# Parskatt/RoMa

Measured on AMD Instinct MI355X. Metric: image-pairs/sec, roma_outdoor 560->864, batch=8 per GPU, higher is better.
Workload: dtype bf16; 1 GPU; roma_outdoor match() 560->864, symmetric, upsample_preds, 8 pairs/GPU/step, seeded synthetic weights + N(0,1) images; precision policy of the reference's bf16 timing script: bfloat16 DINOv2 + float16 autocast for VGG / decoder / refiners (ROMA_MIXED), f32 accumulate; precision_policy=mixed, global_batch=8, streams_per_gpu=2, parallelism=single GPU, outputs_finite=True

## Files before the change

roma_amd/csrc/dwconv_ring.hip:

```cpp
#include <stdlib.h>

#include <algorithm>

#include "elementwise.h"
#include "tuning.h"
#include "gemm.h"

namespace roma {

typedef __attribute__((ext_vector_type(2))) float f32x2;
#define ROMA_LDS __attribute__((address_space(3)))
typedef ROMA_LDS unsigned char lds_u8;

__device__ __attribute__((aligned(256))) unsigned int g_dwr_zero_page[64];

constexpr int DWR_ROWB = 3072;
constexpr int DWR_PXW = 16;
constexpr int DWR_NR = 6;
constexpr int DWR_RING = 4 * DWR_NR * DWR_ROWB;
static_assert(3 * (DWR_NR - 1) + 4 * (DWR_NR - 1) <= 63, "vmcnt is a 6-bit counter");
static_assert(2 * DWR_RING <= 160 * 1024, "two workgroups per CU");

#define ROMA_DWR_WAIT_VM(N) asm volatile("s_waitcnt vmcnt(%0)" ::"n"(N) : "memory")

__device__ __forceinline__ void dwr_glds16(const char* src, lds_u8* lds_wave_base) {
  __builtin_amdgcn_global_load_lds((const __attribute__((address_space(1))) void*)src, (ROMA_LDS void*)lds_wave_base, 16, 0, 0);
}

__device__ __forceinline__ void dwr_read(unsigned long long (&cr)[8], unsigned rd) {
  asm volatile(
      "ds_read_b64 %0, %8\n\tds_read_b64 %1, %8 offset:128\n\tds_read_b64 %2, %8 offset:256\n\t"
      "ds_read_b64 %3, %8 offset:384\n\tds_read_b64 %4, %8 offset:640\n\tds_read_b64 %5, %8 offset:768\n\t"
      "ds_read_b64 %6, %8 offset:896\n\tds_read_b64 %7, %8 offset:1024"
      : "=&v"(cr[0]), "=&v"(cr[1]), "=&v"(cr[2]), "=&v"(cr[3]), "=&v"(cr[4]), "=&v"(cr[5]), "=&v"(cr[6]), "=&v"(cr[7])
      : "v"(rd)
      : "memory");
}
__device__ __forceinline__ void dwr_wait(unsigned long long (&cr)[8]) {
  asm volatile("s_waitcnt lgkmcnt(0)"
               : "+v"(cr[0]), "+v"(cr[1]), "+v"(cr[2]), "+v"(cr[3]), "+v"(cr[4]), "+v"(cr[5]), "+v"(cr[6]), "+v"(cr[7])::"memory");
}

__device__ __forceinline__ void dwr_row(f32x2 (&acc)[5][4][2], const f32x4 (&wreg)[25], f32x2 bias0, f32x2 bias1,
                                        unsigned long long (&cr)[8], unsigned rd_next, bool store, bf16_t* orow, long Cp, int npx) {
  f32x2 v[8][2];
#define ROMA_DWR_CVT(J)                                                  \
  {                                                                      \
    const uint32_t lo_ = (uint32_t)cr[J], hi_ = (uint32_t)(cr[J] >> 32); \
    v[J][0] = f32x2{h16_lo(lo_), h16_hi(lo_)};                           \
    v[J][1] = f32x2{h16_lo(hi_), h16_hi(hi_)};                           \
  }
  ROMA_DWR_CVT(0) ROMA_DWR_CVT(1) ROMA_DWR_CVT(2) ROMA_DWR_CVT(3) ROMA_DWR_CVT(4) ROMA_DWR_CVT(5) ROMA_DWR_CVT(6) ROMA_DWR_CVT(7)
#undef ROMA_DWR_CVT
#pragma unroll
  for (int j = 0; j < 8; ++j) asm volatile("" : "+v"(v[j][0]), "+v"(v[j][1]));
  dwr_read(cr, rd_next);
#pragma unroll
  for (int kx = 0; kx < 5; ++kx) {
    __builtin_amdgcn_sched_barrier(0);
#pragma unroll
    for (int k = 0; k < 5; ++k) {
      const f32x4 wx = wreg[(4 - k) * 5 + kx];
      const f32x2 w0 = f32x2{wx[0], wx[1]}, w1 = f32x2{wx[2], wx[3]};
#pragma unroll
      for (int px = 0; px < 4; ++px) {
        acc[k][px][0] = v[px + kx][0] * w0 + (k == 4 && kx == 0 ? bias0 : acc[k][px][0]);
        acc[k][px][1] = v[px + kx][1] * w1 + (k == 4 && kx == 0 ? bias1 : acc[k][px][1]);
      }
    }
    __builtin_amdgcn_sched_barrier(0);
  }
  if (store) {
#pragma unroll
    for (int px = 0; px < 4; ++px) {
      if (px < npx) {
        uint2 u;
        u.x = pack_relu_h16x2(acc[0][px][0][0], acc[0][px][0][1]);
        u.y = pack_relu_h16x2(acc[0][px][1][0], acc[0][px][1][1]);
        *reinterpret_cast<uint2*>(orow + (long)px * Cp) = u;
      }
    }
  }
#pragma unroll
  for (int k = 0; k < 4; ++k)
#pragma unroll
    for (int px = 0; px < 4; ++px) {
      acc[k][px][0] = acc[k + 1][px][0];
      acc[k][px][1] = acc[k + 1][px][1];
    }
  dwr_wait(cr);
}

__global__ __launch_bounds__(256, 2) void dwconv5x5_ring_kernel(const bf16_t* __restrict__ in, bf16_t* __restrict__ out,
                                                                const float* __restrict__ w, const float* __restrict__ bias,
                                                                int B, int H, int W, int Cp, int SY, int nchunk, int nxg,
                                                                long ntasks) {
  constexpr int NR = DWR_NR;
  __shared__ __attribute__((aligned(1024))) unsigned char ring[DWR_RING];
  const long nwg = (ntasks + 3) / 4, wg_per_xcd = (nwg + 7) / 8;
  const long lw = (long)(blockIdx.x % 8) * wg_per_xcd + blockIdx.x / 8;
  const int lane = threadIdx.x & 63;
  const int wv = __builtin_amdgcn_readfirstlane((int)(threadIdx.x >> 6));
  const long task = lw * 4 + wv;
  if (lw >= nwg || task >= ntasks) return;
  const int xg = (int)(task % nxg);
  long r = task / nxg;
  const int chunk = (int)(r % nchunk);
  r /= nchunk;
  const int yt = (H + SY - 1) / SY;
  const int ys = (int)(r % yt) * SY;
  const int b = (int)(r / yt);
  const int sy = min(SY, H - ys);
  const int T = sy + 4;

  const int cg = lane & 15, xq = lane >> 4;
  const int c = chunk * 64 + cg * 4;

  f32x4 wreg[25];
#pragma unroll
  for (int t = 0; t < 25; ++t) wreg[t] = *reinterpret_cast<const f32x4*>(w + (long)t * Cp + c);
  const f32x4 bx = *reinterpret_cast<const f32x4*>(bias + c);
#pragma unroll
  for (int t = 0; t < 25; ++t) asm volatile("" : "+v"(wreg[t]));
  const f32x2 bias0 = f32x2{bx[0], bx[1]}, bias1 = f32x2{bx[2], bx[3]};
  asm volatile("s_waitcnt vmcnt(0)" ::: "memory");

  const int xb = xg * DWR_PXW + xq * 4;
  const int x0 = xg * DWR_PXW - 2;
  const int npx = min(4, W - xb);

  const char* zsrc = reinterpret_cast<const char*>(g_dwr_zero_page);
  const char* inb = reinterpret_cast<const char*>(in + ((long)b * H * W) * Cp) + (long)chunk * 128;
  const long pitch = (long)W * Cp * 2;
  const __amdgpu_buffer_rsrc_t rs_in = __builtin_amdgcn_make_buffer_rsrc(const_cast<char*>(inb), 0, (int)((long)H * pitch - (long)chunk * 128), 0x00020000);
  unsigned voff[3];
#pragma unroll
  for (int i = 0; i < 3; ++i) {
    const int p = 64 * i + lane, s = p >> 3, part = p & 7;
    const int x = x0 + s - s / 5;
    const bool ok = (s % 5 != 4) && x >= 0 && x < W;
    voff[i] = ok ? (unsigned)(x * Cp * 2 + part * 16) : 0x80000000u;
  }
  unsigned vout = 0x80000000u;
  asm volatile("" : "+v"(vout));
  lds_u8* const myring = (lds_u8*)ring + wv * (NR * DWR_ROWB);
#define ROMA_DWR_BL16(VOFF, SOFF, DST) \
  __builtin_amdgcn_raw_ptr_buffer_load_lds(rs_in, (ROMA_LDS void*)(DST), 16, (int)(VOFF), (int)(SOFF), 0, 0)
#define ROMA_DWR_ISSUE(RROW, SLOT)                                                         \
  {                                                                                        \
    const int yy_ = ys - 2 + (RROW);                                                       \
    if ((RROW) < T && yy_ >= 0 && yy_ < H) {                             \
      const int so_ = yy_ * (int)pitch;                                                    \
      _Pragma("unroll") for (int i = 0; i < 3; ++i) ROMA_DWR_BL16(voff[i], so_, myring + (SLOT) * DWR_ROWB + i * 1024); \
    } else {                                                                               \
      _Pragma("unroll") for (int i = 0; i < 3; ++i) ROMA_DWR_BL16(vout, 0, myring + (SLOT) * DWR_ROWB + i * 1024); \
    }                                                                                      \
  }

  f32x2 acc[5][4][2];
#pragma unroll
  for (int s5 = 0; s5 < 5; ++s5)
#pragma unroll
    for (int px = 0; px < 4; ++px) {
      acc[s5][px][0] = bias0;
      acc[s5][px][1] = bias1;
    }
  const unsigned ring_lds = (unsigned)(size_t)myring;
  const unsigned rd0 = ring_lds + (unsigned)(xq * 5 * 128 + cg * 8);
  bf16_t* const obase = out + ((long)b * H * W) * Cp + c;

#pragma unroll
  for (int rr = 0; rr < NR - 1; ++rr) ROMA_DWR_ISSUE(rr, rr);
  unsigned long long cr[8];
  ROMA_DWR_WAIT_VM(3 * (NR - 2));
  dwr_read(cr, rd0);
  dwr_wait(cr);

  int slot1 = 1;
  int fill = NR - 1;
  bf16_t* orow = obase + ((long)ys * W + xb) * Cp;
  const long orow_step = (long)W * Cp;
#pragma nounroll
  for (int t = 0; t < T; ++t) {
    ROMA_DWR_ISSUE(t + NR - 1, fill);
    ROMA_DWR_WAIT_VM(3 * (NR - 2));
    const bool st = t >= 4;
    dwr_row(acc, wreg, bias0, bias1, cr, rd0 + (unsigned)slot1 * DWR_ROWB, st && npx > 0, orow, (long)Cp, npx);
    if (st) orow += orow_step;
    fill = fill + 1 == NR ? 0 : fill + 1;
    slot1 = slot1 + 1 == NR ? 0 : slot1 + 1;
  }
#undef ROMA_DWR_ISSUE
  ROMA_DWR_WAIT_VM(0);
}

int dwconv5x5_ring_try_launch(const void* in, void* out, const float* w, const float* bias, int B, int H, int W, int Cp, int dt,
                              hipStream_t s) {
  const int dw_ring = tuning(SW_DW_RING);
  if (!dw_ring) return 1;
  if (dt != DT_BF16 || Cp % 64 != 0 || Cp < 256 || H < 1 || W < 1) return 1;
  if ((long)H * W * Cp * 2 >= (1l << 31)) return 1;
  if ((reinterpret_cast<uintptr_t>(in) & 15) != 0 || (reinterpret_cast<uintptr_t>(out) & 7) != 0) return 1;
  if ((reinterpret_cast<uintptr_t>(w) & 15) != 0 || (reinterpret_cast<uintptr_t>(bias) & 15) != 0) return 1;
  const int nchunk = Cp / 64;
  const int nxg = (W + DWR_PXW - 1) / DWR_PXW;
  int SY = H;
  {
    long best = -1;
    const long per_strip = (long)B * nxg * nchunk;
    const int max_sy = std::max(6, (int)tuning(SW_DWR_MAXSY));
    for (int ns = (H + max_sy - 1) / max_sy; ns <= std::max(1, H / 6); ++ns) {
      const int sy = (H + ns - 1) / ns;
      const long nt = per_strip * ((H + sy - 1) / sy);
      const long cost = ((nt + 2047) / 2048) * (sy + 7);
      if (best < 0 || cost < best) {
        best = cost;
        SY = sy;
      }
    }
  }
  const long ntasks = (long)B * ((H + SY - 1) / SY) * nxg * nchunk;
  ROMA_REQUIRE(ntasks < (1l << 31), "dwconv5x5: grid too large");
  const long min_elems = tuning(SW_DW_RING_MINELEMS);
  if (dw_ring != 2 && (long)B * H * W * Cp < min_elems) return 1;
  ProfScope ps("dwconv5x5_kernel<" ROMA_H16_NAME ">", 2.0 * (double)B * H * W * Cp * 2.0, "byte", s);
  const long nwg = (ntasks + 3) / 4;
  hipLaunchKernelGGL(dwconv5x5_ring_kernel, dim3((unsigned)(((nwg + 7) / 8) * 8)), dim3(256), 0, s, (const bf16_t*)in,
                     (bf16_t*)out, w, bias, B, H, W, Cp, SY, nchunk, nxg, ntasks);
  ROMA_LAUNCH_CHECK();
  return 0;
}

}
```

roma_amd/csrc/elementwise.h:

```cpp
#pragma once
#include "common.h"

namespace roma {

int layernorm_launch(const float* x, const float* w, const float* b, void* out, long M, int D, float eps,
                     int dt_out, hipStream_t s);
int layernorm_launch_dt(const void* x, int dt_in, const float* w, const float* b, void* out, long M, int D, float eps,
                        int dt_out, hipStream_t s);

int conv3x3_c3_launch(const float* img, const float* w, const float* bias, void* out, int B, int H, int W,
                      int dt_out, hipStream_t s);

int im2col3x3_c3_launch(const float* img, void* out, int B, int H, int W, int dt_out, hipStream_t s);

int maxpool2x2_launch(const void* in, void* out, int B, int H, int W, int C, int dt, hipStream_t s);

int im2col_patch14_launch(const float* img, void* out, int B, int H, int W, int Kpad, int dt_out, hipStream_t s);

int assemble_tokens_launch(const float* patch, const float* cls, const float* pos, float* tokens, int B, int T,
                           int D, hipStream_t s);

int copy2d_launch(const void* in, long ldi, int dt_in, void* out, long ldo, int dt_out, long rows, int cols,
                  hipStream_t s);

int convert_from_bf16_launch(const void* in, void* out, long n, hipStream_t s);

int rownorm_launch(const void* in, long ld, int dt, float* norms, long M, int C, hipStream_t s);

int gp_basis_launch(const float* w, const float* b, float* Ft, int Dg, int h, int wdt, int npad, hipStream_t s, int copies = 1,
                    long stride = 0);

int transpose_launch(const float* in, float* out, int n, long ld, int batch, hipStream_t s, long stride_in = 0, long stride_out = 0);

int chol_diag_launch(float* A, long ld, long strideA, float* Linv, float* LinvT, int k, int nblk, int batch,
                     hipStream_t s);

int chol_col_launch(float* A, long ld, long strideA, float* LT, long strideLT, int n, int d, float* Linv, float* LinvT, int k,
                    int nblk, int batch, unsigned epoch, int use_leader, hipStream_t s);
int chol_col_restore_launch(float* A, long ld, long strideA, const float* LT, long strideLT, int n, int batch, hipStream_t s);

int pad_identity_launch(float* A, long ld, long strideA, int n, int npad, int batch, hipStream_t s);

int cls_to_flow_launch(const float* logits, long ld, float* flow, float* cert, long M, hipStream_t s);

struct RefinerInputArgs {
  const void* feat = nullptr;
  long ldf = 0;
  const float* flow = nullptr;
  void* d = nullptr;
  long ldd = 0;
  const float* emb_w = nullptr;
  const float* emb_b = nullptr;
  int B = 0, H = 0, W = 0, C = 0, E = 0, Kcorr = 0, nimg = 0, shift = 0;
  float disp_scale = 1.f;
  int dt = 0;
};
int refiner_input_launch(const RefinerInputArgs& a, hipStream_t s);

int dwconv5x5_launch(const void* in, void* out, const float* w, const float* bias, int B, int H, int W, int Cp,
                     int dt, hipStream_t s);
int dwconv5x5_ring_try_launch(const void* in, void* out, const float* w, const float* bias, int B, int H, int W, int Cp, int dt,
                              hipStream_t s);

int refiner_out_launch(const void* d, long ldd, int dt, const float* w , const float* b ,
                       float* flow, float* cert, long M, int Cp, float sx, float sy, hipStream_t s);
int refiner_apply_delta_launch(const float* delta, float* flow, float* cert, long M, float sx, float sy, hipStream_t s);

int resize_bilinear_launch(const float* in, float* out, int B, int Hin, int Win, int Hout, int Wout, int nc,
                           hipStream_t s);

struct FinalArgs {
  const float* flow = nullptr;
  const float* cert = nullptr;
  const float* cert16 = nullptr;
  float* warp = nullptr;
  float* certainty = nullptr;
  int B = 0, H = 0, W = 0, h16 = 0, w16 = 0, symmetric = 1;
};
int final_epilogue_launch(const FinalArgs& a, hipStream_t s);

int checksum_cols_launch(const void* p, long rows, int ld, int c0, int c1, unsigned long long* out, hipStream_t s);
int checksum_launch(const void* p, size_t bytes, unsigned long long* out, hipStream_t s);

}
```

roma_amd/csrc/tuning.hip:

```cpp
#include "tuning.h"

#include <stdlib.h>
#include <string.h>

#include "../../include/roma_hip.h"

namespace roma {
void set_error(const std::string& msg);
namespace {

struct Row {
  Switch id;
  const char* key;
  const char* env;
  long def;
  int floor;
  const char* doc;
};

constexpr Row ROWS[] = {
    {SW_GEMM8P, "gemm8p", "ROMA_GEMM8P", 1, 0, "large bf16 GEMMs on the 8-phase 256 x 256 kernel (1) or on the one-barrier-per-slab kernel (0)"},
    {SW_GEMM_DBG, "gemm_dbg", "ROMA_GEMM_DBG", 0, 0, "experiment bits of the GEMM kernels (1 skip output stores, 2 skip the K loop, 2048 no streaming stores, ...)"},
    {SW_GEMM8P_WALK, "gemm8p_walk", nullptr, -1, 1, "gemm8p: tile rows per group of the persistent walk (1 = row major); unset = 8 from 24 tile columns on, else 1"},
    {SW_GEMM8P_SCHED, "gemm8p_sched", "ROMA_GEMM8P_SCHED", 1, 0, "gemm8p K-loop schedule: 1 k-half phases, 0 quadrant phases (tools builds only)"},
    {SW_GEMM8P_MAXWG, "gemm8p_maxwg", nullptr, -1, 8, "gemm8p, measurement only: cap the persistent grid at n workgroups (a multiple of 8); unset = one per CU"},
    {SW_WS1X1, "ws1x1", "ROMA_WS1X1", 1, 0, "N = K = 576 refiner 1x1 on the weight-stationary kernel (1) or on the 256 x 192 tile kernel (0)"},
    {SW_LC_MODE, "lc_mode", "ROMA_LC_MODE", 0, 0, "local correlation: 0 tiled form + gather work list, 1 every tile on the gather list (key only), 2 per-pixel kernel"},
    {SW_LC_BIN, "lc_bin", "ROMA_LC_BIN", 1, 0, "local correlation: queries of incoherent tiles sorted by target bin, counters in LDS (1) or device atomics (2), or gathered per query (0)"},
    {SW_CONV64, "conv64", "ROMA_CONV64", 7, 0, "weight-stationary VGG front end, bit mask: 1 the Cin = 64 kernels, 2 the Cin = 128 kernel, 4 the fused first layer"},
    {SW_CONV_PATCH, "conv_patch", "ROMA_CONV_PATCH", 1, 0, "patch-resident 3x3 kernel for slab-major VGG layers (1) or gemm8p (0); environment 0 also packs tap-major weights"},
    {SW_ATTN_XCD, "attn_xcd", "ROMA_ATTN_XCD", 1, 0, "attention work items in per-XCD bands of (batch, head) (1) or in plain order (0)"},
    {SW_ATTN_EXP2, "attn_exp2", nullptr, -1, 0, "tools only: force the 2^x softmax of the 16-bit attention kernel on / off; unset = as the caller says"},
    {SW_DW_RING, "dw_ring", "ROMA_DW_RING", 1, 0, "depthwise 5x5: 0 register-prefetch kernel, 1 ring kernel for the large launches, 2 ring kernel for every shape it takes"},
    {SW_GP_COL, "gp_col", "ROMA_GP_COL", 1, 0, "GP Cholesky left-looking, one launch per block column (1) or the right-looking launch chain (0)"},
    {SW_POOL_PROJ, "pool_proj", "ROMA_POOL_PROJ", 1, 0, "max-pool + proj head of strides 1 / 2 in one pass (1) or as separate kernels (0)"},
    {SW_GP_COL_LEADER, "gp_col_leader", "ROMA_GP_COL_LEADER", 1, 0, "block-column Cholesky: a leader workgroup factorises the diagonal block, its product formed one launch ahead (1) or in its own launch (2), or every workgroup its own copy (0)"},
    {SW_GEMM8P_MINM, nullptr, "ROMA_GEMM8P_MINM", 2048, 0, "gemm8p: smallest M it takes for the wide (N >= 2048) dense launches"},
    {SW_GEMM_NT, nullptr, "ROMA_GEMM_NT", 1, 0, "non-temporal output stores in the 16-bit GEMM row writer"},
    {SW_GEMM_F32_FILL, nullptr, "ROMA_GEMM_F32_FILL", 1, 0, "exact-f32 GEMMs below 192 tiles of 256 x 256 run on 128 x 128 tiles"},
    {SW_GEMM_SMALLM, nullptr, "ROMA_GEMM_SMALLM", 1, 0, "GEMMs below 320 tiles of 128 x 128 run on 128 x 64 tiles"},
    {SW_CONV64_SY, nullptr, "ROMA_CONV64_SY", 0, 0, "conv64 strip height in rows; 0 = the split of H with the fewest rounds"},
    {SW_CONV_KORDER, nullptr, "ROMA_CONV_KORDER", 1, 0, "VGG layers with Cout >= 256 pack slab-major weight rows (read when a handle is created)"},
    {SW_RB_SY, nullptr, "ROMA_RB_SY", 0, 0, "fused refiner block strip height in rows; 0 = the split of H with the fewest rounds"},
    {SW_DWR_MAXSY, nullptr, "ROMA_DWR_MAXSY", 1 << 20, 0, "depthwise ring kernel: cap of the strip height in rows (at least 6)"},
    {SW_DW_RING_MINELEMS, nullptr, "ROMA_DW_RING_MINELEMS", 64l << 20, 0, "dw_ring = 1: smallest launch, in elements, that goes to the ring kernel"},
    {SW_RI_VEC, nullptr, "ROMA_RI_VEC", 1, 0, "refiner_input on the 16-byte vector kernel where alignment allows"},
    {SW_OUT_ROW, nullptr, "ROMA_OUT_ROW", 1, 0, "refiner_out: row kernel for C = 24 in 16-bit storage"},
    {SW_OUT_LPR, nullptr, "ROMA_OUT_LPR", 1, 0, "refiner_out, 16-bit: lanes per row chosen to fill the 16-byte pieces best"},
    {SW_OUT_ROWS_IT, nullptr, "ROMA_OUT_ROWS_IT", 0, 0, "refiner_out: row groups per wave (even, >= 2); otherwise 8"},
    {SW_GP_AUG, nullptr, "ROMA_GP_AUG", 1, 0, "GP Cholesky: right-hand sides stored behind A ride along the factorisation (0 = separate forward loop)"},
    {SW_GP_BWD2, nullptr, "ROMA_GP_BWD2", 1, 0, "GP Cholesky: backward substitution with one launch per step (0 = two)"},
    {SW_COMPOSE_OUT, nullptr, "ROMA_COMPOSE_OUT", 1, 0, "initial value of the handle option compose_out_conv (read when a handle is created)"},
    {SW_VIT_RES_F32, nullptr, "ROMA_VIT_RES_F32", 0, 0, "force DINOv2's f32 residual stream in the 16-bit modes"},
    {SW_STREAMS, nullptr, "ROMA_STREAMS", 0, 0, "number of sub-batch streams of match(); 0 = the handle's option"},
    {SW_STREAMS_SERIAL, nullptr, "ROMA_STREAMS_SERIAL", 0, 0, "diagnostic: sub-batch streams run one after the other"},
    {SW_DEBUG_DUAL_SLOT, nullptr, "ROMA_DEBUG_DUAL_SLOT", -1, 0, "diagnostic: keep the stream split in debug mode, sub-batch k captures the stages of ROMA_DEBUG_ONLY"},
};
constexpr int NROWS = sizeof(ROWS) / sizeof(ROWS[0]);
constexpr bool rows_in_enum_order() {
  for (int i = 0; i < NROWS; ++i)
    if (ROWS[i].id != i) return false;
  return true;
}
static_assert(NROWS == SW_COUNT && rows_in_enum_order(), "one row per Switch, in enum order");
constexpr bool json_plain(const char* s) {
  for (; s && *s; ++s)
    if (*s == '"' || *s == '\\' || *s < ' ') return false;
  return true;
}
constexpr bool rows_json_plain() {
  for (const Row& r : ROWS)
    if (!json_plain(r.key) || !json_plain(r.env) || !json_plain(r.doc)) return false;
  return true;
}
static_assert(rows_json_plain(), "keys, environment names and docs: plain ASCII without quote, backslash or control character");

struct Overrides {
  long v[SW_COUNT];
  constexpr Overrides() : v{} {
    for (long& x : v) x = -1;
  }
};
[[clang::require_constant_initialization]] Overrides g_override;

struct Env {
  long v[SW_COUNT];
  Env() {
    for (int i = 0; i < NROWS; ++i) {
      const char* s = ROWS[i].env ? getenv(ROWS[i].env) : nullptr;
      v[i] = s ? atol(s) : ROWS[i].def;
    }
  }
};
const Env& env() {
  static const Env e;
  return e;
}

}

long tuning_env(Switch id) { return env().v[id]; }
long tuning_override(Switch id) { return g_override.v[id] >= ROWS[id].floor ? g_override.v[id] : -1; }
long tuning(Switch id) { return g_override.v[id] >= ROWS[id].floor ? g_override.v[id] : tuning_env(id); }

int tuning_set(const char* key, long value) {
  for (const Row& r : ROWS)
    if (r.key && !strcmp(r.key, key)) {
      g_override.v[r.id] = value >= r.floor ? value : -1;
      return 0;
    }
  set_error(std::string("roma_tuning: unknown key ") + key);
  return ROMA_ERR_ARG;
}

std::string tuning_describe() {
  std::string js = "[";
  for (const Row& r : ROWS) {
    const auto quoted = [](const char* s) { return s ? "\"" + std::string(s) + "\"" : std::string("null"); };
    const long ov = tuning_override(r.id);
    js += std::string(r.id ? ", " : "") + "{\"key\": " + quoted(r.key) + ", \"env\": " + quoted(r.env) +
          ", \"default\": " + std::to_string(r.def) + ", \"override\": " + (ov >= 0 ? std::to_string(ov) : "null") +
          ", \"value\": " + std::to_string(tuning(r.id)) + ", \"doc\": " + quoted(r.doc) + "}";
  }
  return js + "]";
}

}
```

Baseline: 108.7 image-pairs/s.

## Add two-channels-per-lane depthwise 5x5 ring kernel for small images

Adds a second ring-buffered depthwise 5x5 kernel in which each lane holds two channels and four pixels. Rows are 8 pixels wide and the kernel uses smaller LDS rings (5 rows of 2 KB per wave), so four workgroups fit per CU. The default dispatch selects it for small images (H*W <= 8192) with large total size, aiming at better occupancy and less halo overhead than the 16-pixel ring kernel. The strip-height search is factored into a helper that takes a residency parameter.

```diff
diff --git a/roma_amd/csrc/dwconv_lanes.hip b/roma_amd/csrc/dwconv_lanes.hip
--- /dev/null
+++ b/roma_amd/csrc/dwconv_lanes.hip
@@ -0,0 +1,188 @@
+#include <stdlib.h>
+
+#include <algorithm>
+
+#include "elementwise.h"
+#include "tuning.h"
+#include "gemm.h"
+
+namespace roma {
+
+typedef __attribute__((ext_vector_type(2))) float f32x2;
+#define ROMA_LDS __attribute__((address_space(3)))
+typedef ROMA_LDS unsigned char lds_u8;
+
+constexpr int DWL_PXW = 8;
+constexpr int DWL_NPX = DWL_PXW + 4;
+constexpr int DWL_ROWB = 2048;
+constexpr int DWL_NR = 5;
+constexpr int DWL_RING = 4 * DWL_NR * DWL_ROWB;
+static_assert(2 * (DWL_NR - 1) + 4 * (DWL_NR - 1) <= 63, "vmcnt is a 6-bit counter");
+static_assert(4 * DWL_RING <= 160 * 1024, "four workgroups per CU");
+static_assert(DWL_NPX * 128 <= DWL_ROWB && DWL_ROWB == 2 * 1024, "a ring row is two DMA instructions of 64 x 16 B");
+
+#define ROMA_DWL_WAIT_VM(N) asm volatile("s_waitcnt vmcnt(%0)" ::"n"(N) : "memory")
+
+__device__ __forceinline__ void dwl_read(unsigned long long (&cr)[4], unsigned rd) {
+  asm volatile(
+      "ds_read2_b32 %0, %4 offset1:32\n\tds_read2_b32 %1, %4 offset0:64 offset1:96\n\t"
+      "ds_read2_b32 %2, %4 offset0:128 offset1:160\n\tds_read2_b32 %3, %4 offset0:192 offset1:224"
+      : "=&v"(cr[0]), "=&v"(cr[1]), "=&v"(cr[2]), "=&v"(cr[3])
+      : "v"(rd)
+      : "memory");
+}
+__device__ __forceinline__ void dwl_wait(unsigned long long (&cr)[4]) {
+  asm volatile("s_waitcnt lgkmcnt(0)" : "+v"(cr[0]), "+v"(cr[1]), "+v"(cr[2]), "+v"(cr[3])::"memory");
+}
+
+__device__ __forceinline__ void dwl_row(f32x2 (&acc)[5][4], const f32x2 (&wreg)[25], f32x2 bias2, unsigned long long (&cr)[4],
+                                        unsigned rd_next, bool store, bf16_t* orow, long Cp, int npx) {
+  f32x2 v[8];
+#pragma unroll
+  for (int j = 0; j < 4; ++j) {
+    const uint32_t lo = (uint32_t)cr[j], hi = (uint32_t)(cr[j] >> 32);
+    v[2 * j] = f32x2{h16_lo(lo), h16_hi(lo)};
+    v[2 * j + 1] = f32x2{h16_lo(hi), h16_hi(hi)};
+  }
+#pragma unroll
+  for (int j = 0; j < 8; ++j) asm volatile("" : "+v"(v[j]));
+  dwl_read(cr, rd_next);
+#pragma unroll
+  for (int kx = 0; kx < 5; ++kx) {
+    __builtin_amdgcn_sched_barrier(0);
+#pragma unroll
+    for (int k = 0; k < 5; ++k) {
+      const f32x2 wx = wreg[(4 - k) * 5 + kx];
+#pragma unroll
+      for (int px = 0; px < 4; ++px)
+        acc[k][px] = v[px + kx] * wx + (k == 4 && kx == 0 ? bias2 : acc[k][px]);
+    }
+    __builtin_amdgcn_sched_barrier(0);
+  }
+  if (store) {
+#pragma unroll
+    for (int px = 0; px < 4; ++px)
+      if (px < npx)
+        *reinterpret_cast<uint32_t*>(orow + (long)px * Cp) = pack_relu_h16x2(acc[0][px][0], acc[0][px][1]);
+  }
+#pragma unroll
+  for (int k = 0; k < 4; ++k)
+#pragma unroll
+    for (int px = 0; px < 4; ++px) acc[k][px] = acc[k + 1][px];
+  dwl_wait(cr);
+}
+
+__global__ __launch_bounds__(256, 4) void dwconv5x5_lanes_kernel(const bf16_t* __restrict__ in, bf16_t* __restrict__ out,
+                                                                 const float* __restrict__ w, const float* __restrict__ bias,
+                                                                 int B, int H, int W, int Cp, int SY, int nchunk, int nxg,
+                                                                 long ntasks) {
+  constexpr int NR = DWL_NR, ROWB = DWL_ROWB;
+  __shared__ __attribute__((aligned(1024))) unsigned char ring[DWL_RING];
+  const long nwg = (ntasks + 3) / 4, wg_per_xcd = (nwg + 7) / 8;
+  const long lw = (long)(blockIdx.x % 8) * wg_per_xcd + blockIdx.x / 8;
+  const int lane = threadIdx.x & 63;
+  const int wv = __builtin_amdgcn_readfirstlane((int)(threadIdx.x >> 6));
+  const long task = lw * 4 + wv;
+  if (lw >= nwg || task >= ntasks) return;
+  const int xg = (int)(task % nxg);
+  long r = task / nxg;
+  const int chunk = (int)(r % nchunk);
+  r /= nchunk;
+  const int yt = (H + SY - 1) / SY;
+  const int ys = (int)(r % yt) * SY;
+  const int b = (int)(r / yt);
+  const int sy = min(SY, H - ys);
+  const int T = sy + 4;
+
+  const int cp = lane & 31, xq = lane >> 5;
+  const int c = chunk * 64 + cp * 2;
+
+  f32x2 wreg[25];
+#pragma unroll
+  for (int t = 0; t < 25; ++t) wreg[t] = *reinterpret_cast<const f32x2*>(w + (long)t * Cp + c);
+  f32x2 bias2 = *reinterpret_cast<const f32x2*>(bias + c);
+#pragma unroll
+  for (int t = 0; t < 25; ++t) asm volatile("" : "+v"(wreg[t]));
+  asm volatile("" : "+v"(bias2));
+  asm volatile("s_waitcnt vmcnt(0)" ::: "memory");
+
+  const int xb = xg * DWL_PXW + xq * 4;
+  const int x0 = xg * DWL_PXW - 2;
+  const int npx = min(4, W - xb);
+
+  const char* inb = reinterpret_cast<const char*>(in + ((long)b * H * W) * Cp) + (long)chunk * 128;
+  const long pitch = (long)W * Cp * 2;
+  const __amdgpu_buffer_rsrc_t rs_in = __builtin_amdgcn_make_buffer_rsrc(const_cast<char*>(inb), 0, (int)((long)H * pitch - (long)chunk * 128), 0x00020000);
+  unsigned voff[2];
+#pragma unroll
+  for (int i = 0; i < 2; ++i) {
+    const int p = 64 * i + lane, px = p >> 3, part = p & 7;
+    const int x = x0 + px;
+    const bool ok = px < DWL_NPX && x >= 0 && x < W;
+    voff[i] = ok ? (unsigned)(x * Cp * 2 + part * 16) : 0x80000000u;
+  }
+  unsigned vout = 0x80000000u;
+  asm volatile("" : "+v"(vout));
+  lds_u8* const myring = (lds_u8*)ring + wv * (NR * ROWB);
+#define ROMA_DWL_BL16(VOFF, SOFF, DST) \
+  __builtin_amdgcn_raw_ptr_buffer_load_lds(rs_in, (ROMA_LDS void*)(DST), 16, (int)(VOFF), (int)(SOFF), 0, 0)
+#define ROMA_DWL_ISSUE(RROW, SLOT)                                                         \
+  {                                                                                        \
+    const int yy_ = ys - 2 + (RROW);                                                       \
+    if ((RROW) < T && yy_ >= 0 && yy_ < H) {                             \
+      const int so_ = yy_ * (int)pitch;                                                    \
+      _Pragma("unroll") for (int i = 0; i < 2; ++i) ROMA_DWL_BL16(voff[i], so_, myring + (SLOT) * ROWB + i * 1024); \
+    } else {                                                                               \
+      _Pragma("unroll") for (int i = 0; i < 2; ++i) ROMA_DWL_BL16(vout, 0, myring + (SLOT) * ROWB + i * 1024); \
+    }                                                                                      \
+  }
+
+  f32x2 acc[5][4];
+#pragma unroll
+  for (int s5 = 0; s5 < 5; ++s5)
+#pragma unroll
+    for (int px = 0; px < 4; ++px) acc[s5][px] = bias2;
+  const unsigned ring_lds = (unsigned)(size_t)myring;
+  const unsigned rd0 = ring_lds + (unsigned)(xq * 4 * 128 + cp * 4);
+  bf16_t* const obase = out + ((long)b * H * W) * Cp + c;
+
+#pragma unroll
+  for (int rr = 0; rr < NR - 1; ++rr) ROMA_DWL_ISSUE(rr, rr);
+  unsigned long long cr[4];
+  ROMA_DWL_WAIT_VM(2 * (NR - 2));
+  dwl_read(cr, rd0);
+  dwl_wait(cr);
+
+  int slot1 = 1;
+  int fill = NR - 1;
+  bf16_t* orow = obase + ((long)ys * W + xb) * Cp;
+  const long orow_step = (long)W * Cp;
+#pragma nounroll
+  for (int t = 0; t < T; ++t) {
+    ROMA_DWL_ISSUE(t + NR - 1, fill);
+    ROMA_DWL_WAIT_VM(2 * (NR - 2));
+    const bool st = t >= 4;
+    dwl_row(acc, wreg, bias2, cr, rd0 + (unsigned)slot1 * ROWB, st && npx > 0, orow, (long)Cp, npx);
+    if (st) orow += orow_step;
+    fill = fill + 1 == NR ? 0 : fill + 1;
+    slot1 = slot1 + 1 == NR ? 0 : slot1 + 1;
+  }
+#undef ROMA_DWL_ISSUE
+  ROMA_DWL_WAIT_VM(0);
+}
+
+int dwconv5x5_lanes_launch(const void* in, void* out, const float* w, const float* bias, int B, int H, int W, int Cp, hipStream_t s) {
+  const int nchunk = Cp / 64;
+  const int nxg = (W + DWL_PXW - 1) / DWL_PXW;
+  const int SY = dwconv5x5_ring_strip_height((long)B * nxg * nchunk, H, 4096);
+  const long ntasks = (long)B * ((H + SY - 1) / SY) * nxg * nchunk;
+  ROMA_REQUIRE(ntasks < (1l << 31), "dwconv5x5: grid too large");
+  ProfScope ps("dwconv5x5_kernel<" ROMA_H16_NAME ">", 2.0 * (double)B * H * W * Cp * 2.0, "byte", s);
+  const long nwg = (ntasks + 3) / 4;
+  hipLaunchKernelGGL(dwconv5x5_lanes_kernel, dim3((unsigned)(((nwg + 7) / 8) * 8)), dim3(256), 0, s, (const bf16_t*)in,
+                     (bf16_t*)out, w, bias, B, H, W, Cp, SY, nchunk, nxg, ntasks);
+  ROMA_LAUNCH_CHECK();
+  return 0;
+}
+
+}
diff --git a/roma_amd/csrc/dwconv_ring.hip b/roma_amd/csrc/dwconv_ring.hip
--- a/roma_amd/csrc/dwconv_ring.hip
+++ b/roma_amd/csrc/dwconv_ring.hip
@@ -194,6 +194,22 @@
   ROMA_DWR_WAIT_VM(0);
 }
 
+int dwconv5x5_ring_strip_height(long per_strip, int H, int resident) {
+  int SY = H;
+  long best = -1;
+  const int max_sy = std::max(6, (int)tuning(SW_DWR_MAXSY));
+  for (int ns = (H + max_sy - 1) / max_sy; ns <= std::max(1, H / 6); ++ns) {
+    const int sy = (H + ns - 1) / ns;
+    const long nt = per_strip * ((H + sy - 1) / sy);
+    const long cost = ((nt + resident - 1) / resident) * (sy + 7);
+    if (best < 0 || cost < best) {
+      best = cost;
+      SY = sy;
+    }
+  }
+  return SY;
+}
+
 int dwconv5x5_ring_try_launch(const void* in, void* out, const float* w, const float* bias, int B, int H, int W, int Cp, int dt,
                               hipStream_t s) {
   const int dw_ring = tuning(SW_DW_RING);
@@ -202,23 +218,11 @@
   if ((long)H * W * Cp * 2 >= (1l << 31)) return 1;
   if ((reinterpret_cast<uintptr_t>(in) & 15) != 0 || (reinterpret_cast<uintptr_t>(out) & 7) != 0) return 1;
   if ((reinterpret_cast<uintptr_t>(w) & 15) != 0 || (reinterpret_cast<uintptr_t>(bias) & 15) != 0) return 1;
+  if (dw_ring == 3 || (dw_ring != 2 && (long)H * W <= 8192 && (long)B * H * W * Cp >= (16l << 20)))
+    return dwconv5x5_lanes_launch(in, out, w, bias, B, H, W, Cp, s);
   const int nchunk = Cp / 64;
   const int nxg = (W + DWR_PXW - 1) / DWR_PXW;
-  int SY = H;
-  {
-    long best = -1;
-    const long per_strip = (long)B * nxg * nchunk;
-    const int max_sy = std::max(6, (int)tuning(SW_DWR_MAXSY));
-    for (int ns = (H + max_sy - 1) / max_sy; ns <= std::max(1, H / 6); ++ns) {
-      const int sy = (H + ns - 1) / ns;
-      const long nt = per_strip * ((H + sy - 1) / sy);
-      const long cost = ((nt + 2047) / 2048) * (sy + 7);
-      if (best < 0 || cost < best) {
-        best = cost;
-        SY = sy;
-      }
-    }
-  }
+  const int SY = dwconv5x5_ring_strip_height((long)B * nxg * nchunk, H, 2048);
   const long ntasks = (long)B * ((H + SY - 1) / SY) * nxg * nchunk;
   ROMA_REQUIRE(ntasks < (1l << 31), "dwconv5x5: grid too large");
   const long min_elems = tuning(SW_DW_RING_MINELEMS);
diff --git a/roma_amd/csrc/elementwise.h b/roma_amd/csrc/elementwise.h
--- a/roma_amd/csrc/elementwise.h
+++ b/roma_amd/csrc/elementwise.h
@@ -61,6 +61,8 @@
                      int dt, hipStream_t s);
 int dwconv5x5_ring_try_launch(const void* in, void* out, const float* w, const float* bias, int B, int H, int W, int Cp, int dt,
                               hipStream_t s);
+int dwconv5x5_lanes_launch(const void* in, void* out, const float* w, const float* bias, int B, int H, int W, int Cp, hipStream_t s);
+int dwconv5x5_ring_strip_height(long per_strip, int H, int resident);
 
 int refiner_out_launch(const void* d, long ldd, int dt, const float* w , const float* b ,
                        float* flow, float* cert, long M, int Cp, float sx, float sy, hipStream_t s);
diff --git a/roma_amd/csrc/tuning.hip b/roma_amd/csrc/tuning.hip
--- a/roma_amd/csrc/tuning.hip
+++ b/roma_amd/csrc/tuning.hip
@@ -31,7 +31,7 @@
     {SW_CONV_PATCH, "conv_patch", "ROMA_CONV_PATCH", 1, 0, "patch-resident 3x3 kernel for slab-major VGG layers (1) or gemm8p (0); environment 0 also packs tap-major weights"},
     {SW_ATTN_XCD, "attn_xcd", "ROMA_ATTN_XCD", 1, 0, "attention work items in per-XCD bands of (batch, head) (1) or in plain order (0)"},
     {SW_ATTN_EXP2, "attn_exp2", nullptr, -1, 0, "tools only: force the 2^x softmax of the 16-bit attention kernel on / off; unset = as the caller says"},
-    {SW_DW_RING, "dw_ring", "ROMA_DW_RING", 1, 0, "depthwise 5x5: 0 register-prefetch kernel, 1 ring kernel for the large launches, 2 ring kernel for every shape it takes"},
+    {SW_DW_RING, "dw_ring", "ROMA_DW_RING", 1, 0, "depthwise 5x5: 0 register-prefetch kernel, 1 a ring kernel where one is faster (large launches; small images on the two-channels-per-lane form), 2 ring kernel for every shape it takes, 3 its two-channels-per-lane form for every shape it takes"},
     {SW_GP_COL, "gp_col", "ROMA_GP_COL", 1, 0, "GP Cholesky left-looking, one launch per block column (1) or the right-looking launch chain (0)"},
     {SW_POOL_PROJ, "pool_proj", "ROMA_POOL_PROJ", 1, 0, "max-pool + proj head of strides 1 / 2 in one pass (1) or as separate kernels (0)"},
     {SW_GP_COL_LEADER, "gp_col_leader", "ROMA_GP_COL_LEADER", 1, 0, "block-column Cholesky: a leader workgroup factorises the diagonal block, its product formed one launch ahead (1) or in its own launch (2), or every workgroup its own copy (0)"},
```

New measurement: 109.2 image-pairs/s (median of 6 runs). Within noise of the previous version (+0.5%).
